# jketterl/digiham

Measured on AMD Instinct MI355X. Metric: concurrent 48 kS/s DMR channels sustained end-to-end (rrc_filter->gfsk_demodulator->dmr_decoder), higher is better.
Workload: dtype f32; 1 GPU; 16384 DMR channels/GPU x 3.96 s (190080 samples) of 48 kS/s FM-discriminator audio, full chain rrc(wide)->gfsk(10)->dmr_decoder incl. BPTC(196,96) (BASELINE con; channels_per_gpu=16384, total_channels=16384

## Files before the change

### digiham_amd/csrc/dsp_core.hpp

```cpp
#pragma once

#include "dh_portable.hpp"
#include "wave_ops.hpp"

#define DH_VARIANCE_SYMBOLS 100
#define DH_VOLUME_RB_SIZE 100
#define DH_FTILE 1024
#define DH_FIR_L 16
#define DH_PF_N 5
#define DH_PF_SINK 512
#define DH_MAX_NZ 160
#define DH_MAX_SPS 40
DH_HD uint32_t dh_history(uint32_t sps) { return DH_VARIANCE_SYMBOLS * (sps > 10u ? sps : 10u) + 152u; }
DH_HD uint32_t dh_tail_max(uint32_t sps) { return 256u + dh_history(sps); }
#define DH_STATE_HDR 32

enum { DH_ST_K = 0, DH_ST_OFF = 1, DH_ST_TAIL = 2, DH_ST_NSYM = 3, DH_ST_ORDERED = 4, DH_ST_BLOCKS = 5,
       DH_ST_P0 = 6,
       DH_ST_CUR_START = 7, DH_ST_CUR_OFF = 8, DH_ST_PREV_START = 9, DH_ST_PREV_OFF = 10,
       DH_ST_BLOCK_FLAGS = 11,
       DH_ST_E_CUR = 12, DH_ST_E_PREV = 13, DH_ST_E_COUNT = 14, DH_ST_E_BLOCK = 15,
       DH_ST_UNCERTAIN = 16, DH_ST_EXACT_RUNS = 17, DH_ST_EXACT_BLOCKS = 18,
       DH_ST_PART = 19,
       DH_ST_DIAG = 20 };
// ... 434 lines not shown
        }
    }
}
#else
template <int NZ, bool ONE>
inline void dh_fir_f16(const float* hw, const uint32_t (*G)[DH_WAVE][4], int lane, float k1, float k2, float* out16) {
    constexpr int DH_F16_KSTEPS = DH_F16_KSTEPS_OF(NZ), DH_F16_H2_OFFSET = DH_F16_H2_OFFSET_OF(NZ);
    const uint16_t* h1 = reinterpret_cast<const uint16_t*>(hw);
    const uint16_t* h2 = reinterpret_cast<const uint16_t*>(hw + DH_F16_H2_OFFSET);
    const int n = lane & 15, g = lane >> 4;
    for (int T = 0; T < 4; T++) for (int r = 0; r < 4; r++) {
        const uint32_t o = DH_F16_OUT(T, r, g, n), b16 = o - (uint32_t) n;
        float mn = 0.0f, sc = 0.0f;
        for (int i = 0; i < 3; i++) {
            const int pass = ONE ? (i == 0 ? 1 : i == 1 ? 0 : 2) : i;
            for (int s = 0; s < DH_F16_KSTEPS; s++) for (int qq = 0; qq < 4; qq++) for (int j = 0; j < 8; j++) {
                const int kk = 8 * qq + j;
                const uint32_t w = G[(pass == 1 ? DH_F16_KSTEPS : 0) + s][16 * qq + n][j >> 1];
                const float tap = dh_f16_value((uint16_t) (w >> (16 * (j & 1))));
                const uint16_t hv = (pass == 2 ? h2 : h1)[b16 + 32u * (uint32_t) s + (uint32_t) kk];
                if (pass == 0 && !ONE) mn = __builtin_fmaf(dh_f16_value(hv), tap, mn); else sc = __builtin_fmaf(dh_f16_value(hv), tap, sc);
            }
        }
        out16[4 * T + r] = ONE ? sc * k1 : __builtin_fmaf(sc, k2, mn * k1);
    }
}
#endif

DH_HD float dh_virtual_sample(const float* tail, uint32_t tc, const float* in, uint32_t idx) {
    return idx < tc ? tail[idx] : in[idx - tc];
}

struct DhAgcPair { float mn0, mx0, mn1, mx1; };

#if DH_ON_GPU
__device__ __forceinline__ void dh_agc_scan(DhDspShared& S, uint32_t k0, uint32_t k1, DH_LANE_STRUCT_REF(DhAgcPair, agc)) {
    const int lane = dh_fresh_lane_id_();
    const uint32_t e0 = 2u * (uint32_t) lane, e1 = e0 + 1u;
    const float c0 = e0 < k0 ? S.vol_old[e0] : S.vol_new[e0];
    const float c1 = e1 < k0 ? S.vol_old[e1] : S.vol_new[e1];
    const bool v0 = e0 < k1, v1 = e1 < k1;
    const float pmn0 = v0 ? c0 : DH_FLT_MAX, pmn1 = v1 ? c1 : DH_FLT_MAX;
    const float pmx0 = v0 ? c0 : DH_FLT_MIN, pmx1 = v1 ? c1 : DH_FLT_MIN;
    float pmn = dh_vmin(pmn0, pmn1), pmx = dh_vmax(pmx0, pmx1);
    const uint32_t r0 = 126u - e0, r1 = r0 + 1u;
    const float o0 = S.vol_old[r0], o1 = S.vol_old[r1];
    const float omn0 = r0 < DH_VOLUME_RB_SIZE ? o0 : DH_FLT_MAX, omn1 = r1 < DH_VOLUME_RB_SIZE ? o1 : DH_FLT_MAX;
    const float omx0 = r0 < DH_VOLUME_RB_SIZE ? o0 : DH_FLT_MIN, omx1 = r1 < DH_VOLUME_RB_SIZE ? o1 : DH_FLT_MIN;
    float smn = dh_vmin(omn0, omn1), smx = dh_vmax(omx0, omx1);
    dh_wave_prefix_minmax2(pmn, pmx, smn, smx);
    float epmn = DH_FLT_MAX, epmx = DH_FLT_MIN, esmn = DH_FLT_MAX, esmx = DH_FLT_MIN;
    dh_wave_prev4(epmn, epmx, esmn, esmx, pmn, pmx, smn, smx);
    const int from = (63 - lane) << 2;
    const float s1n = __int_as_float(__builtin_amdgcn_ds_bpermute(from, __float_as_int(esmn)));
    const float s1x = __int_as_float(__builtin_amdgcn_ds_bpermute(from, __float_as_int(esmx)));
    const float s0n = __int_as_float(__builtin_amdgcn_ds_bpermute(from, __float_as_int(dh_vmin(omn1, esmn))));
    const float s0x = __int_as_float(__builtin_amdgcn_ds_bpermute(from, __float_as_int(dh_vmax(omx1, esmx))));
    DhAgcPair r;
    r.mn0 = dh_vmin(dh_vmin(epmn, pmn0), s0n); r.mx0 = dh_vmax(dh_vmax(epmx, pmx0), s0x);
    r.mn1 = dh_vmin(pmn, s1n); r.mx1 = dh_vmax(pmx, s1x);
    S.mn[e0] = r.mn0; S.mx[e0] = r.mx0; S.mn[e1] = r.mn1; S.mx[e1] = r.mx1;
    agc = r;
}
#else
inline void dh_agc_scan(DhDspShared& S, uint32_t k0, uint32_t k1, DH_LANE_STRUCT_REF(DhAgcPair, agc)) {
    float pmn = DH_FLT_MAX, pmx = DH_FLT_MIN;
    for (uint32_t j = 0; j < k0; j++) { pmn = dh_fmin_(pmn, S.vol_old[j]); pmx = dh_fmax_(pmx, S.vol_old[j]); }
    for (uint32_t k = k0; k < k1; k++) {
        pmn = dh_fmin_(pmn, S.vol_new[k]); pmx = dh_fmax_(pmx, S.vol_new[k]);
        float smn = DH_FLT_MAX, smx = DH_FLT_MIN;
        for (uint32_t j = k + 1; j < DH_VOLUME_RB_SIZE; j++) { smn = dh_fmin_(smn, S.vol_old[j]); smx = dh_fmax_(smx, S.vol_old[j]); }
        S.mn[k] = dh_fmin_(pmn, smn); S.mx[k] = dh_fmax_(pmx, smx);
    }
    for (uint32_t l = 0; l < DH_WAVE; l++) {
        const uint32_t e0 = 2u * l, e1 = e0 + 1u, a = e0 >= k0 && e0 < k1 ? e0 : k0, b = e1 >= k0 && e1 < k1 ? e1 : k0;
        agc[l] = DhAgcPair{ S.mn[a], S.mx[a], S.mn[b], S.mx[b] };
    }
}
#endif

template <int NZ, bool FAST, int SPS> struct DhIsBounded {
    static constexpr bool value = !FAST && ((NZ == 80 && SPS == 10) || (NZ == 160 && SPS != 10));
};
#ifndef DH_STOP_AFTER
#define DH_STOP_AFTER 99
#endif
#define DH_BOUND_T_FACTOR 3.5f
#define DH_BOUND_XMAX_LO 1e-25f
#define DH_BOUND_XMAX_HI 1e15f

inline float dh_fir_error_coefficient(const float* taps_half, uint32_t nz, double gain) {
    double l1 = 0.0;
    for (uint32_t i = 0; i <= nz; i++) { const double c = taps_half[i <= nz / 2 ? i : nz - i]; l1 += c < 0 ? -c : c; }
    const double kappa = nz == 80 ? 240.0 : 1.44 * (2.0 * (nz + 1) + 5.0);
    const double coef = kappa * 5.9604644775390625e-08 * l1 / (gain < 0 ? -gain : gain) * 1.0001;
    float f = (float) coef;
    if ((double) f < coef) { union { float f; uint32_t u; } b; b.f = f; b.u++; f = b.f; }
    return f;
}

template <int NZ>
DH_HD float dh_exact_filtered(const float* tail, uint32_t tc, const float* in, uint32_t nv, const float* tapsf, double gain, double rgain, int32_t f) {
    if (f < 0 || (uint32_t) f + (uint32_t) NZ >= nv) return 0.0f;
    float acc = 0.0f;
// ... 182 lines not shown
            DH_FOR_LANES_FRESH(lane) {
                const uint32_t e = r * DH_WAVE + (uint32_t) lane;
                if (e < nj * nrows) {
                    uint32_t jj, i;
                    if (full) { jj = e / sps; i = e - jj * sps; }
                    else {
                        const uint32_t c = e / nj;
                        jj = e - c * nj;
                        uint64_t m = rows & all;
                        for (uint32_t b = 0; b < c; b++) m &= m - 1;
                        i = (uint32_t) dh_ffs64(m);
                    }
                    const uint32_t j = j0 + jj;
                    const int32_t f = C.cur_start + (int32_t) (j * sps) + (j ? C.cur_off : 0) + (int32_t) i;
                    S.var_rb[i * DH_VARIANCE_SYMBOLS + j] = dh_exact_filtered_lds<NZ>(stage, base, C.nv, C.tapsf, C.gain, C.rgain, f);
                }
            }
        }
    }
    DH_BARRIER();
}

template <int NZ>
DH_COLD void dh_exact_fir_pass(const DhDspParams& P, DhDspShared& S, uint32_t need, DH_LANE_ARRAY(float, (&fo), DH_FIR_L)) {
    float tv[NZ / 2 + 1];
    for (int i = 0; i <= NZ / 2; i++) tv[i] = S.tapsf[i];
    DH_FOR_LANES_FRESH(lane) {
        if ((uint32_t) (lane * DH_FIR_L) < need) {
            dh_fir_lane<NZ, false, false, true>(tv, P.gain, P.rgain, P.inv_gain, S.xf, lane, DH_LA(fo, lane));
        }
    }
}

template <int SPS>
DH_HD void dh_symbol_windows(DhDspShared& S, const float* fbuf, uint32_t k0, uint32_t m, int32_t step_off, uint32_t sps, uint32_t ev_lo, uint32_t ev_hi, float sps_rcp) {
#define DH_FB(n) fbuf[n]
    if (SPS == 10 && DH_STOP_AFTER >= 3) DH_FOR_LANES_FRESH(lane) {
        const uint32_t l = (uint32_t) lane;
        const uint32_t qa = l + 1u, qb = l < 35u ? l + 65u : 0u;
        const bool va = qa < m, vb = l < 35u ? qb < m : l == 35u;
        const float* srca = fbuf + (int32_t) (qa * 10u) + step_off;
        const float* srcb = l < 35u ? srca + 640 : fbuf;
        float v[10], w[10];
        dh_lds_run10_pair(srca, srcb, v, w);
        float vola = v[0], volb = w[0];
#pragma unroll
        for (int i = 1; i < 10; i++) { vola += v[i]; volb += w[i]; }
        const float mida = ((v[3] + v[4]) + v[5]) + v[6], midb = ((w[3] + w[4]) + w[5]) + w[6];
        const float volume_a = dh_div_const(vola, 10.0f, sps_rcp), volume_b = dh_div_const(volb, 10.0f, sps_rcp);
        if (va) {
            const uint32_t ka = k0 + qa;
            dh_lds_store_row10<0>(S.var_rb + ka, v[0], v[1], v[2], v[3], v[4], v[5], v[6], v[7], v[8], v[9]);
            S.sum[qa] = mida; S.vol_new[ka] = volume_a;
        }
        if (vb) {
            const uint32_t kb = k0 + qb;
            dh_lds_store_row10<0>(S.var_rb + kb, w[0], w[1], w[2], w[3], w[4], w[5], w[6], w[7], w[8], w[9]);
            S.sum[qb] = midb; S.vol_new[kb] = volume_b;
        }
        dh_lds_stores_done();
    }
    if (SPS == 20 && DH_STOP_AFTER >= 3) DH_FOR_LANES_FRESH(lane) {
        const uint32_t l = (uint32_t) lane;
        const uint32_t q = l < 63u ? l + 1u : 0u;
        const bool valid = q < m;
        const float* src = valid && q > 0u ? fbuf + (int32_t) (q * 20u) + step_off : fbuf;
        float v[20];
        dh_lds_run<20>(src, v);
        float vol = v[0];
#pragma unroll
        for (int i = 1; i < 20; i++) vol += v[i];
        const float mid = ((((v[7] + v[8]) + v[9]) + v[10]) + v[11]) + v[12];
        const float volume = dh_div_const(vol, 20.0f, sps_rcp);
        if (valid) {
            const uint32_t k = k0 + q;
            dh_lds_store_row10<0>(S.var_rb + k, v[0], v[1], v[2], v[3], v[4], v[5], v[6], v[7], v[8], v[9]);
            dh_lds_store_row10<1000>(S.var_rb + k, v[10], v[11], v[12], v[13], v[14], v[15], v[16], v[17], v[18], v[19]);
            S.sum[q] = mid; S.vol_new[k] = volume;
        }
        dh_lds_stores_done();
    }
    if (SPS == 40 && DH_STOP_AFTER >= 3) DH_FOR_LANES_FRESH(lane) {
        const uint32_t l = (uint32_t) lane;
        const uint32_t q = l < 63u ? l + 1u : 0u;
        const bool valid = q < m;
        const float* src = valid && q > 0u ? fbuf + (int32_t) (q * 40u) + step_off : fbuf;
        float v[40];
        dh_lds_run<40>(src, v);
        float vol = v[0], mid = v[13];
#pragma unroll
        for (int i = 1; i < 40; i++) vol += v[i];
#pragma unroll
        for (int i = 14; i < 27; i++) mid += v[i];
// ... 301 lines not shown
                        DH_BALLOT_ACC(v_above, l > hmin, lane);
                        DH_BALLOT_ACC(v_ok, DH_LA(iv_ok, lane)[0] != 0u, lane);
                        DH_BALLOT_ACC(v_pos, l > 0.0f, lane);
                        DH_BALLOT_ACC(v_small, h < 4999999.0f, lane);
                        DH_BALLOT_ACC(v_big, l > 5000001.0f, lane);
                    }
                    const uint64_t phases = sps >= 64u ? ~0ull : ((1ull << sps) - 1ull);
                    const uint64_t cand = ~v_above & phases;
                    const bool one = cand != 0 && (cand & (cand - 1)) == 0;
                    const bool sure = one && (v_ok & phases) == phases && (((v_pos & cand) && (v_small & cand)) || (v_big & cand));
                    if (!sure) continue;
                    DH_FOR_LANES_FRESH(lane) { if (DH_IS_LANE0(lane)) S.stats[1]++; }
                    const uint32_t vmin_pos = (uint32_t) dh_ffs64(cand);
                    if (v_big & cand) {
                    } else if (vmin_pos > 0 && vmin_pos < sps / 2) new_off = +1;
                    else if (vmin_pos >= sps / 2 && vmin_pos < sps - 1) new_off = -1;
                    break;
                }
                double vmin = S.variance[0]; uint32_t vmin_pos = 0;
                for (uint32_t i = 1; i < sps; i++) if (S.variance[i] < vmin) { vmin = S.variance[i]; vmin_pos = i; }
                DH_FOR_LANES_FRESH(lane) { if (DH_IS_LANE0(lane)) S.stats[1]++; }
                if (vmin <= 0 || vmin > 5000000) {
                } else if (vmin_pos > 0 && vmin_pos < sps / 2) new_off = +1;
                else if (vmin_pos >= sps / 2 && vmin_pos < sps - 1) new_off = -1;
                break;
            }
        }
    }
    return new_off;
}

struct DhSliceSetup { bool four_levels, e_pos, width_pow2, pair_store; float T_eff, inv_width; };
template <int SPS, int LV, bool BOUNDED>
DH_HD void dh_slice_symbols(const DhDspParams& P, DhDspShared& S, DH_LANE_STRUCT_IN(DhAgcPair, agc), uint8_t* out, uint32_t k0, uint32_t m, uint32_t ev_lo, uint32_t ev_hi,
                            const DhSliceSetup& U, uint64_t& vote_a, uint64_t& vote_b) {
    const bool four_levels = U.four_levels, e_pos = U.e_pos, width_pow2 = U.width_pow2, pair_store = U.pair_store;
    const float T_eff = U.T_eff, inv_width = U.inv_width;
    DH_FOR_LANES_FRESH(lane) {
        const uint32_t qa = 2u * (uint32_t) lane;
        const bool va = qa < m, vb = qa + 1u < m;
        const uint32_t qq = va ? qa : 0u, k = k0 + qq;
        const DhAgcPair& own = DH_LS(agc, lane);
        dh_f2 mn, mx;
        if (k0 == 0u) { mn = dh_f2_make(own.mn0, own.mn1); mx = dh_f2_make(own.mx0, own.mx1); }
        else { mn = dh_f2_make(S.mn[k], S.mn[k + 1u]); mx = dh_f2_make(S.mx[k], S.mx[k + 1u]); }
        const dh_f2 sumq = dh_f2_make(S.sum[qq], S.sum[qq + 1u]);
        const dh_f2 center = dh_f2_scale(dh_f2_add(mx, mn), 0.5f);
        const dh_f2 average = width_pow2 ? dh_f2_scale(sumq, inv_width) : SPS == 20 ? dh_div_const2(sumq, 6.0f, inv_width)
                                                                                    : dh_f2_make(sumq.x / (float) (ev_hi - ev_lo), sumq.y / (float) (ev_hi - ev_lo));
        const dh_f2 c625 = dh_f2_make(0.625f, 0.625f);
        const dh_f2 umid = dh_f2_fma(dh_f2_sub(mx, center), c625, center);
        const dh_f2 lmid = dh_f2_fma(dh_f2_sub(mn, center), c625, center);
        const bool above_a = average.x > center.x, above_b = average.y > center.y;
        const uint8_t sym4a = above_a ? (average.x > umid.x ? 1 : 0) : (average.x < lmid.x ? 3 : 2);
        const uint8_t sym4b = above_b ? (average.y > umid.y ? 1 : 0) : (average.y < lmid.y ? 3 : 2);
        const uint8_t sym2a = LV == 4 ? (uint8_t) 0 : above_a ? (uint8_t) !P.invert : (uint8_t) (P.invert != 0);
        const uint8_t sym2b = LV == 4 ? (uint8_t) 0 : above_b ? (uint8_t) !P.invert : (uint8_t) (P.invert != 0);
        const uint8_t sa = four_levels ? sym4a : sym2a, sb = four_levels ? sym4b : sym2b;
        bool doubt_a = false, doubt_b = false;
        if (BOUNDED) {
            const dh_f2 du = dh_f2_sub(average, umid), dl = dh_f2_sub(average, lmid), dc = dh_f2_sub(average, center);
            const float da = dh_min3_abs(four_levels ? du.x : DH_FLT_MAX, four_levels ? dl.x : DH_FLT_MAX, dc.x);
            const float db = dh_min3_abs(four_levels ? du.y : DH_FLT_MAX, four_levels ? dl.y : DH_FLT_MAX, dc.y);
            doubt_a = va && e_pos && !(da > T_eff);
            doubt_b = vb && e_pos && !(db > T_eff);
        }
#ifdef DH_IGNORE_DOUBT
        doubt_a = false; doubt_b = false;
#endif
        if (DH_LIKELY(pair_store)) {
            if (vb) *reinterpret_cast<uint16_t*>(out + qa) = (uint16_t) ((uint32_t) sa | ((uint32_t) sb << 8));
            if (DH_UNLIKELY((m & 1u) != 0u)) { if (qa + 1u == m) out[qa] = sa; }
        } else {
            if (va) out[qa] = sa;
            if (vb) out[qa + 1u] = sb;
        }
        DH_BALLOT_ACC(vote_a, doubt_a, lane);
        DH_BALLOT_ACC(vote_b, doubt_b, lane);
    }
// ... 439 lines not shown
        DH_TAPFRAG_SETTLE(tapfrag_regs, NFRAG, MF16);
        DH_PHASE_MARK(1);
        const float* fbuf = S.xf;

        const uint32_t p_next = last_start + sps + ((k0 == 0 && m == 1) ? (uint32_t) step_off : 0u);
        const uint32_t pf_have = dh_min<uint32_t>(DH_FTILE + NZ, nv - p_next);
        DH_LANE_ARRAY(dh_f4, pfr, PF_REG ? DH_PF_N : 1);
        const bool pf_plain = p_next - tc < pf_lim;
        const bool pf_reg = PF_REG && pf_plain && P.exact_mode != 2;
        if constexpr (KEEPF) {
            const uint32_t f_lo = tc > (uint32_t) NZ ? tc - (uint32_t) NZ : 0u;
            const uint32_t s0 = p < f_lo ? f_lo - p : 0u;
            const uint32_t s1 = dh_min<uint32_t>(p_next - p, nf > p ? nf - p : 0u);
            float* orow = P.filt_out + (size_t) ch * P.filt_stride + ((ptrdiff_t) p + (ptrdiff_t) NZ - (ptrdiff_t) tc);
            DH_FOR_LANES_FRESH(lane) {
                for (uint32_t e = s0 + (uint32_t) lane; e < s1; e += DH_WAVE) orow[e] = fbuf[e];
            }
        }

        DH_COMPILER_FENCE();
        float e_blk = 0.0f;
        if (BOUNDED) { e_blk = dh_uniform_f(__builtin_fmaxf(e_blk_run, e_run)); e_blk_run = e_blk; }
        const float e_eff = BOUNDED ? dh_uniform_f(__builtin_fmaxf(e_run, __builtin_fmaxf(e_cur, e_prev))) : 0.0f;
        const float T = DH_BOUND_T_FACTOR * e_eff;
        uint64_t vote_a = 0, vote_b = 0;
        const bool four_levels = LV ? LV == 4 : P.levels == 4;
        const bool force_doubt = BOUNDED && P.exact_mode == 1;
        const bool e_pos = e_eff > 0.0f || force_doubt;
        const float T_eff = force_doubt ? __builtin_inff() : T;
        const float inv_width = 1.0f / (float) (ev_hi - ev_lo);
        const bool width_pow2 = ((ev_hi - ev_lo) & (ev_hi - ev_lo - 1u)) == 0u;
        const bool pair_store = ((uint32_t) (uintptr_t) syms + nsym) % 2u == 0u;

        dh_symbol_windows<SPS>(S, fbuf, k0, m, step_off, sps, ev_lo, ev_hi, sps_rcp);
        DH_BARRIER();
        DH_PHASE_MARK(2);

        dh_issue_next_window<NZ, PF_REG>(S, in, tc, p_next, pf_plain, pf_reg, pfr);

        DH_LANE_STRUCT(DhAgcPair, agc) = {};
        if (DH_STOP_AFTER >= 4) dh_agc_scan(S, k0, k0 + m, agc);
        DH_BARRIER();
        DH_PHASE_MARK(3);

        if (DH_STOP_AFTER >= 5) {
            const DhSliceSetup U = { four_levels, e_pos, width_pow2, pair_store, T_eff, inv_width };
            dh_slice_symbols<SPS, LV, BOUNDED>(P, S, agc, syms + nsym, k0, m, ev_lo, ev_hi, U, vote_a, vote_b);
        }
        if (BOUNDED && DH_UNLIKELY((vote_a | vote_b) != 0)) {
            dh_settle_doubts<NZ>(P, S, BS, V, syms + nsym, k0, e_eff, sps, ev_lo, ev_hi, vote_a, vote_b);
        }

        DH_PHASE_MARK(4);
        int32_t new_off = 0;
        const bool block_done = (k0 + m == DH_VARIANCE_SYMBOLS);
        if (block_done && DH_STOP_AFTER >= 6) {
            new_off = dh_timing_decision<NZ, SPS, BOUNDED>(P, S, BS, V, sps, k0, e_blk);
        }

        DH_PHASE_MARK(5);
        DH_FOR_LANES_FRESH(lane) {
            const uint32_t ka = k0 + (uint32_t) lane, kb = ka + DH_WAVE, ke = k0 + m;
            const uint32_t ia = ka < ke ? ka : k0, ib = kb < ke ? kb : k0;
            const float va_ = S.vol_new[ia], vb_ = S.vol_new[ib];
            S.vol_old[ia] = va_;
            S.vol_old[ib] = vb_;
        }
        staged_p = 0xFFFFFFFFu;
        if (DH_LIKELY(pf_reg)) {
            if constexpr (PF_REG && MF16) { if (DH_LIKELY((dh_stage_f16<NZ, ONE_CHAIN>(P, S, pfr, pf_have, st_e_run, st_k1, st_k2)))) staged_p = p_next; }
            else if constexpr (PF_PLAIN) {
                static_assert(!PF_PLAIN || (DH_FTILE == 4u * DH_WAVE * (DH_PF_N - 1)), "four full groups cover the window");
                DH_FOR_LANES_FRESH(lane) {
                    const uint32_t l4 = 4u * (uint32_t) lane;
                    float* ldst = &S.xf[l4];
#pragma unroll
                    for (int r = 0; r < DH_PF_N - 1; r++) {
                        dh_f4 w = DH_LA(pfr, lane)[PF_REG ? r : 0];
                        if (DH_UNLIKELY(pf_have < DH_FTILE)) w = dh_zero_beyond(w, l4 + 4u * DH_WAVE * (uint32_t) r, pf_have);
                        dh_store4(ldst + 4 * DH_WAVE * r, w);
// ... 185 lines not shown
```

### digiham_amd/csrc/wave_ops.hpp

```cpp
#pragma once

#include "dh_portable.hpp"

#define DH_FLT_MAX 3.402823466e+38f
#define DH_DBL_MAX 1.7976931348623157e+308
#define DH_FLT_MIN 1.175494351e-38f

#if DH_ON_GPU
typedef float dh_f2 __attribute__((ext_vector_type(2)));
typedef float dh_v4f __attribute__((ext_vector_type(4)));
typedef float dh_f32x4 __attribute__((ext_vector_type(4)));
typedef _Float16 dh_h8 __attribute__((ext_vector_type(8)));
typedef _Float16 dh_h4 __attribute__((ext_vector_type(4)));
typedef uint32_t dh_u4 __attribute__((ext_vector_type(4)));
#else
struct dh_f2 { float x, y; };
typedef uint16_t dh_h4[4];
#endif
struct __attribute__((aligned(4))) dh_f4 { float x, y, z, w; };
struct alignas(16) dh_f4a { float x, y, z, w; };
DH_HD dh_f4 dh_load4_unaligned(const float* p) { dh_f4 v; __builtin_memcpy(&v, p, sizeof(v)); return v; }
DH_HD void dh_store4(float* q, const dh_f4& v) { q[0] = v.x; q[1] = v.y; q[2] = v.z; q[3] = v.w; }
DH_HD void dh_store4_unaligned(float* q, const dh_f4& v) { __builtin_memcpy(q, &v, sizeof(v)); }

// ... 144 lines not shown
    dh_v4f xs; xs.x = v.x; xs.y = v.y; xs.z = v.z; xs.w = v.w;
    xs = xs * scale;
    const dh_h4 a = __builtin_convertvector(xs, dh_h4);
    const dh_v4f af = __builtin_convertvector(a, dh_v4f);
    const dh_f2 x01 = xs.xy, x23 = xs.zw, a01 = af.xy, a23 = af.zw;
    dh_f2 r01, r23;
    asm("v_pk_add_f32 %0, %1, %2 neg_lo:[0,1] neg_hi:[0,1]" : "=v"(r01) : "v"(x01), "v"(a01));
    asm("v_pk_add_f32 %0, %1, %2 neg_lo:[0,1] neg_hi:[0,1]" : "=v"(r23) : "v"(x23), "v"(a23));
    dh_v4f r; r.xy = r01; r.zw = r23;
    h1 = a; h2 = __builtin_convertvector(r, dh_h4);
#else
    const float x[4] = { v.x, v.y, v.z, v.w };
    for (int i = 0; i < 4; i++) {
        const float xs = x[i] * scale;
        h1[i] = dh_f16_bits(xs);
        h2[i] = dh_f16_bits(xs - dh_f16_value(h1[i]));
    }
#endif
}
DH_HD void dh_h4_store(dh_h4* dst, const dh_h4& v) { __builtin_memcpy(dst, &v, sizeof(dh_h4)); }

#if DH_ON_GPU
template <int O0, int O1> __device__ __forceinline__ dh_f2 dh_lds_read2(uint32_t addr) {
    static_assert(O0 < 256 && O1 < 256, "ds_read2_b32 offsets are 8-bit dword counts");
    dh_f2 v;
    asm volatile("ds_read2_b32 %0, %1 offset0:%2 offset1:%3" : "=v"(v) : "v"(addr), "n"(O0), "n"(O1) : "memory");
    return v;
}
template <int OFF_BYTES> __device__ __forceinline__ dh_f2 dh_lds_read_b64(uint32_t addr) {
    dh_f2 v;
    asm volatile("ds_read_b64 %0, %1 offset:%2" : "=v"(v) : "v"(addr), "n"(OFF_BYTES) : "memory");
    return v;
}
template <int OFF_BYTES> __device__ __forceinline__ dh_v4f dh_lds_read_b128(uint32_t addr) {
    dh_v4f v;
    asm volatile("ds_read_b128 %0, %1 offset:%2" : "=v"(v) : "v"(addr), "n"(OFF_BYTES) : "memory");
    return v;
}
#endif
template <int N> DH_HD void dh_lds_run(const float* src, float (&v)[N]) {
#if DH_ON_GPU
    static_assert(N == 20 || N == 40, "five or ten 16-byte reads");
    const uint32_t a = (uint32_t) (uintptr_t) (const __attribute__((address_space(3))) float*) src;
    dh_v4f x0 = dh_lds_read_b128<0>(a), x1 = dh_lds_read_b128<16>(a), x2 = dh_lds_read_b128<32>(a), x3 = dh_lds_read_b128<48>(a), x4 = dh_lds_read_b128<64>(a);
    if constexpr (N == 20) {
        asm volatile("s_waitcnt lgkmcnt(0)" : "+v"(x0), "+v"(x1), "+v"(x2), "+v"(x3), "+v"(x4) :: "memory");
        v[0] = x0.x; v[1] = x0.y; v[2] = x0.z; v[3] = x0.w; v[4] = x1.x; v[5] = x1.y; v[6] = x1.z; v[7] = x1.w; v[8] = x2.x; v[9] = x2.y;
        v[10] = x2.z; v[11] = x2.w; v[12] = x3.x; v[13] = x3.y; v[14] = x3.z; v[15] = x3.w; v[16] = x4.x; v[17] = x4.y; v[18] = x4.z; v[19] = x4.w;
    } else {
        dh_v4f x5 = dh_lds_read_b128<80>(a), x6 = dh_lds_read_b128<96>(a), x7 = dh_lds_read_b128<112>(a), x8 = dh_lds_read_b128<128>(a), x9 = dh_lds_read_b128<144>(a);
        asm volatile("s_waitcnt lgkmcnt(0)" : "+v"(x0), "+v"(x1), "+v"(x2), "+v"(x3), "+v"(x4), "+v"(x5), "+v"(x6), "+v"(x7), "+v"(x8), "+v"(x9) :: "memory");
        const dh_v4f x[10] = { x0, x1, x2, x3, x4, x5, x6, x7, x8, x9 };
#pragma unroll
        for (int i = 0; i < 10; i++) { v[4 * i] = x[i].x; v[4 * i + 1] = x[i].y; v[4 * i + 2] = x[i].z; v[4 * i + 3] = x[i].w; }
    }
#else
    for (int i = 0; i < N; i++) v[i] = src[i];
#endif
}
DH_HD void dh_lds_run10_pair(const float* srca, const float* srcb, float (&v)[10], float (&w)[10]) {
#if DH_ON_GPU
    const uint32_t aa = (uint32_t) (uintptr_t) (const __attribute__((address_space(3))) float*) srca;
    const uint32_t ab = (uint32_t) (uintptr_t) (const __attribute__((address_space(3))) float*) srcb;
    dh_f2 x0 = dh_lds_read_b64<0>(aa), x1 = dh_lds_read_b64<8>(aa), x2 = dh_lds_read_b64<16>(aa), x3 = dh_lds_read_b64<24>(aa), x4 = dh_lds_read_b64<32>(aa);
    dh_f2 y0 = dh_lds_read_b64<0>(ab), y1 = dh_lds_read_b64<8>(ab), y2 = dh_lds_read_b64<16>(ab), y3 = dh_lds_read_b64<24>(ab), y4 = dh_lds_read_b64<32>(ab);
    asm volatile("s_waitcnt lgkmcnt(0)" : "+v"(x0), "+v"(x1), "+v"(x2), "+v"(x3), "+v"(x4), "+v"(y0), "+v"(y1), "+v"(y2), "+v"(y3), "+v"(y4) :: "memory");
    v[0] = x0.x; v[1] = x0.y; v[2] = x1.x; v[3] = x1.y; v[4] = x2.x; v[5] = x2.y; v[6] = x3.x; v[7] = x3.y; v[8] = x4.x; v[9] = x4.y;
    w[0] = y0.x; w[1] = y0.y; w[2] = y1.x; w[3] = y1.y; w[4] = y2.x; w[5] = y2.y; w[6] = y3.x; w[7] = y3.y; w[8] = y4.x; w[9] = y4.y;
#else
    for (int i = 0; i < 10; i++) { v[i] = srca[i]; w[i] = srcb[i]; }
#endif
}

#if DH_ON_GPU
template <int OFF_WORDS> __device__ __forceinline__ void dh_lds_store4_at(float* base, const dh_f4& v) {
    static_assert(4 * OFF_WORDS + 12 < 65536, "ds_write_b32 offsets are 16-bit byte counts");
    const uint32_t addr = (uint32_t) (uintptr_t) (__attribute__((address_space(3))) float*) base;
    asm volatile("ds_write_b32 %0, %1 offset:%5\n\tds_write_b32 %0, %2 offset:%6\n\tds_write_b32 %0, %3 offset:%7\n\tds_write_b32 %0, %4 offset:%8"
                 :: "v"(addr), "v"(v.x), "v"(v.y), "v"(v.z), "v"(v.w), "n"(4 * OFF_WORDS), "n"(4 * OFF_WORDS + 4), "n"(4 * OFF_WORDS + 8), "n"(4 * OFF_WORDS + 12) : "memory");
}
__device__ __forceinline__ void dh_lds_stores_done() { asm volatile("s_waitcnt lgkmcnt(0)" ::: "memory"); }
template <int K> __device__ __forceinline__ void dh_lds_store_row10(float* base, float a0, float a1, float a2, float a3, float a4, float a5, float a6, float a7, float a8, float a9) {
    const uint32_t addr = (uint32_t) (uintptr_t) (__attribute__((address_space(3))) float*) base;
    asm volatile("ds_write_b32 %0, %1 offset:%11\n\tds_write_b32 %0, %2 offset:%12\n\tds_write_b32 %0, %3 offset:%13\n\tds_write_b32 %0, %4 offset:%14\n\t"
                 "ds_write_b32 %0, %5 offset:%15\n\tds_write_b32 %0, %6 offset:%16\n\tds_write_b32 %0, %7 offset:%17\n\tds_write_b32 %0, %8 offset:%18\n\t"
                 "ds_write_b32 %0, %9 offset:%19\n\tds_write_b32 %0, %10 offset:%20"
                 :: "v"(addr), "v"(a0), "v"(a1), "v"(a2), "v"(a3), "v"(a4), "v"(a5), "v"(a6), "v"(a7), "v"(a8), "v"(a9),
                    "n"(4 * K), "n"(4 * (K + 100)), "n"(4 * (K + 200)), "n"(4 * (K + 300)), "n"(4 * (K + 400)), "n"(4 * (K + 500)), "n"(4 * (K + 600)),
                    "n"(4 * (K + 700)), "n"(4 * (K + 800)), "n"(4 * (K + 900)) : "memory");
}
#else
template <int OFF_WORDS> inline void dh_lds_store4_at(float* base, const dh_f4& v) { dh_store4(base + OFF_WORDS, v); }
inline void dh_lds_stores_done() {}
template <int K> inline void dh_lds_store_row10(float* base, float a0, float a1, float a2, float a3, float a4, float a5, float a6, float a7, float a8, float a9) {
    const float a[10] = { a0, a1, a2, a3, a4, a5, a6, a7, a8, a9 };
    for (int i = 0; i < 10; i++) base[i * 100 + K] = a[i];
}
#endif

DH_HD void dh_l2_touch_lines(const float* base, uint32_t n, float* sink) {
#if DH_ON_GPU
    const uint32_t pf_lane = (uint32_t) dh_fresh_lane_id_();
    const float* line = base + 32u * pf_lane;
    const uint32_t sink_addr = (uint32_t) (uintptr_t) (__attribute__((address_space(3))) float*) sink;
    uint32_t keep_m0;
    if (32u * pf_lane < n)
        asm volatile("s_mov_b32 %0, m0\n\ts_mov_b32 m0, %1\n\tglobal_load_lds_dword %2, off\n\ts_mov_b32 m0, %0"
                     : "=&s"(keep_m0) : "s"(sink_addr), "v"(line) : "memory");
#endif
}
DH_HD void dh_global_loads_done() { DH_GPU_ELSE(asm volatile("s_waitcnt vmcnt(0)" ::: "memory"), (void) 0); }

#if DH_ON_GPU
#define DH_TAPFRAG_REGS(name, N, table) dh_u4 name[N]
#define DH_TAPFRAG_LOAD(name, N, table, on) do { if constexpr (on) { const dh_u4* tf_ = reinterpret_cast<const dh_u4*>(table) + dh_fresh_lane_id_(); \
        _Pragma("unroll") for (int f_ = 0; f_ < (N); f_++) name[f_] = tf_[DH_WAVE * f_]; } } while (0)
#define DH_TAPFRAG_SETTLE(name, N, on) do { if constexpr (on) { _Pragma("unroll") for (int f_ = 0; f_ < (N); f_++) \
        asm volatile("" :: "v"(name[f_])); } } while (0)
#else
#define DH_TAPFRAG_REGS(name, N, table) const uint32_t (* const name)[DH_WAVE][4] = reinterpret_cast<const uint32_t (*)[DH_WAVE][4]>(table)
#define DH_TAPFRAG_LOAD(name, N, table, on) ((void) 0)
#define DH_TAPFRAG_SETTLE(name, N, on) ((void) 0)
#endif

#if DH_ON_GPU
__device__ __forceinline__ void dh_wave_prefix_minmax2(float& mn, float& mx, float& mn2, float& mx2) {
// ... 103 lines not shown
```

Baseline: 13.98 million channels.

## Keep SPS10 symbol windows in lane registers, drop barriers before AGC scan and slicing

For the 10-samples-per-symbol path, each lane now handles two adjacent symbols from one contiguous 20-sample LDS read and keeps their volume, mid-sum and matching old-volume values in registers. These feed the AGC scan and the slicer directly, so the two block barriers between window, AGC and slice stages are removed. Stores are merged into paired ds_write2 instructions. This adds a cold shift of symbol 0 when step_off is nonzero and fallback LDS reads when k0 is not zero, and correctness now depends on lane ownership matching across the stages.

```diff
diff --git a/digiham_amd/csrc/dsp_core.hpp b/digiham_amd/csrc/dsp_core.hpp
--- a/digiham_amd/csrc/dsp_core.hpp
+++ b/digiham_amd/csrc/dsp_core.hpp
@@ -490,19 +490,30 @@
 }
 
 struct DhAgcPair { float mn0, mx0, mn1, mx1; };
+struct DhWinPair { float vol0, vol1, sum0, sum1, old0, old1; };
 
 #if DH_ON_GPU
-__device__ __forceinline__ void dh_agc_scan(DhDspShared& S, uint32_t k0, uint32_t k1, DH_LANE_STRUCT_REF(DhAgcPair, agc)) {
+template <bool PAIRS>
+__device__ __forceinline__ void dh_agc_scan(DhDspShared& S, uint32_t k0, uint32_t k1, DH_LANE_STRUCT_REF(DhAgcPair, agc), DH_LANE_STRUCT_IN(DhWinPair, win), bool from_win) {
     const int lane = dh_fresh_lane_id_();
     const uint32_t e0 = 2u * (uint32_t) lane, e1 = e0 + 1u;
-    const float c0 = e0 < k0 ? S.vol_old[e0] : S.vol_new[e0];
-    const float c1 = e1 < k0 ? S.vol_old[e1] : S.vol_new[e1];
+    float c0, c1;
+    if (!PAIRS) { c0 = e0 < k0 ? S.vol_old[e0] : S.vol_new[e0]; c1 = e1 < k0 ? S.vol_old[e1] : S.vol_new[e1]; }
+    else if (DH_LIKELY(from_win)) { c0 = win.vol0; c1 = win.vol1; }
+    else {
+        c0 = dh_lds_read_b32<0>(dh_lds_addr((e0 < k0 ? S.vol_old : S.vol_new) + e0));
+        c1 = dh_lds_read_b32<0>(dh_lds_addr((e1 < k0 ? S.vol_old : S.vol_new) + e1));
+        dh_lds_reads_done(c0, c1);
+    }
     const bool v0 = e0 < k1, v1 = e1 < k1;
     const float pmn0 = v0 ? c0 : DH_FLT_MAX, pmn1 = v1 ? c1 : DH_FLT_MAX;
     const float pmx0 = v0 ? c0 : DH_FLT_MIN, pmx1 = v1 ? c1 : DH_FLT_MIN;
     float pmn = dh_vmin(pmn0, pmn1), pmx = dh_vmax(pmx0, pmx1);
     const uint32_t r0 = 126u - e0, r1 = r0 + 1u;
-    const float o0 = S.vol_old[r0], o1 = S.vol_old[r1];
+    float o0, o1;
+    if (!PAIRS) { o0 = S.vol_old[r0]; o1 = S.vol_old[r1]; }
+    else if (DH_LIKELY(from_win)) { o0 = win.old0; o1 = win.old1; }
+    else { o0 = dh_lds_read_b32<0>(dh_lds_addr(S.vol_old + r0)); o1 = dh_lds_read_b32<0>(dh_lds_addr(S.vol_old + r1)); dh_lds_reads_done(o0, o1); }
     const float omn0 = r0 < DH_VOLUME_RB_SIZE ? o0 : DH_FLT_MAX, omn1 = r1 < DH_VOLUME_RB_SIZE ? o1 : DH_FLT_MAX;
     const float omx0 = r0 < DH_VOLUME_RB_SIZE ? o0 : DH_FLT_MIN, omx1 = r1 < DH_VOLUME_RB_SIZE ? o1 : DH_FLT_MIN;
     float smn = dh_vmin(omn0, omn1), smx = dh_vmax(omx0, omx1);
@@ -521,13 +532,18 @@
     agc = r;
 }
 #else
-inline void dh_agc_scan(DhDspShared& S, uint32_t k0, uint32_t k1, DH_LANE_STRUCT_REF(DhAgcPair, agc)) {
+template <bool PAIRS>
+inline void dh_agc_scan(DhDspShared& S, uint32_t k0, uint32_t k1, DH_LANE_STRUCT_REF(DhAgcPair, agc), DH_LANE_STRUCT_IN(DhWinPair, win), bool from_win) {
     float pmn = DH_FLT_MAX, pmx = DH_FLT_MIN;
     for (uint32_t j = 0; j < k0; j++) { pmn = dh_fmin_(pmn, S.vol_old[j]); pmx = dh_fmax_(pmx, S.vol_old[j]); }
     for (uint32_t k = k0; k < k1; k++) {
-        pmn = dh_fmin_(pmn, S.vol_new[k]); pmx = dh_fmax_(pmx, S.vol_new[k]);
+        const float vk = !from_win ? S.vol_new[k] : (k & 1u) ? win[k >> 1].vol1 : win[k >> 1].vol0;
+        pmn = dh_fmin_(pmn, vk); pmx = dh_fmax_(pmx, vk);
         float smn = DH_FLT_MAX, smx = DH_FLT_MIN;
-        for (uint32_t j = k + 1; j < DH_VOLUME_RB_SIZE; j++) { smn = dh_fmin_(smn, S.vol_old[j]); smx = dh_fmax_(smx, S.vol_old[j]); }
+        for (uint32_t j = k + 1; j < DH_VOLUME_RB_SIZE; j++) {
+            const float oj = !from_win ? S.vol_old[j] : (j & 1u) ? win[(127u - j) >> 1].old1 : win[(126u - j) >> 1].old0;
+            smn = dh_fmin_(smn, oj); smx = dh_fmax_(smx, oj);
+        }
         S.mn[k] = dh_fmin_(pmn, smn); S.mx[k] = dh_fmax_(pmx, smx);
     }
     for (uint32_t l = 0; l < DH_WAVE; l++) {
@@ -776,33 +792,43 @@
     }
 }
 
+DH_COLD void dh_shift_symbol0(float* fbuf, int32_t step_off) {
+    DH_LANE_VALUE(float, t);
+    DH_FOR_LANES_FRESH(lane) { DH_LV(t, lane) = fbuf[lane < 10 ? lane : 0]; }
+    DH_FOR_LANES_FRESH(lane) { if (lane < 10) fbuf[lane + step_off] = DH_LV(t, lane); }
+}
+
 template <int SPS>
-DH_HD void dh_symbol_windows(DhDspShared& S, const float* fbuf, uint32_t k0, uint32_t m, int32_t step_off, uint32_t sps, uint32_t ev_lo, uint32_t ev_hi, float sps_rcp) {
+DH_HD void dh_symbol_windows(DhDspShared& S, const float* fbuf, uint32_t k0, uint32_t m, int32_t step_off, uint32_t sps, uint32_t ev_lo, uint32_t ev_hi, float sps_rcp,
+                             DH_LANE_STRUCT_REF(DhWinPair, win)) {
 #define DH_FB(n) fbuf[n]
     if (SPS == 10 && DH_STOP_AFTER >= 3) DH_FOR_LANES_FRESH(lane) {
         const uint32_t l = (uint32_t) lane;
-        const uint32_t qa = l + 1u, qb = l < 35u ? l + 65u : 0u;
-        const bool va = qa < m, vb = l < 35u ? qb < m : l == 35u;
-        const float* srca = fbuf + (int32_t) (qa * 10u) + step_off;
-        const float* srcb = l < 35u ? srca + 640 : fbuf;
-        float v[10], w[10];
-        dh_lds_run10_pair(srca, srcb, v, w);
+        const uint32_t qa = 2u * l, qb = qa + 1u;
+        const bool vb = qb < m;
+        const float* src = l < 50u ? fbuf + (int32_t) (l * 20u) + step_off : fbuf;
+        float x[20], v[10], w[10], old0, old1;
+        dh_lds_run20_with_pair(src, x, S.vol_old + (126u - qa), old0, old1);
+#pragma unroll
+        for (int i = 0; i < 10; i++) { v[i] = x[i]; w[i] = x[10 + i]; }
         float vola = v[0], volb = w[0];
 #pragma unroll
         for (int i = 1; i < 10; i++) { vola += v[i]; volb += w[i]; }
-        const float mida = ((v[3] + v[4]) + v[5]) + v[6], midb = ((w[3] + w[4]) + w[5]) + w[6];
+        float mida = v[3] + v[4]; DH_TO_VGPR(mida); mida += v[5]; DH_TO_VGPR(mida); mida += v[6]; DH_TO_VGPR(mida);
+        const float midb = ((w[3] + w[4]) + w[5]) + w[6];
         const float volume_a = dh_div_const(vola, 10.0f, sps_rcp), volume_b = dh_div_const(volb, 10.0f, sps_rcp);
-        if (va) {
-            const uint32_t ka = k0 + qa;
-            dh_lds_store_row10<0>(S.var_rb + ka, v[0], v[1], v[2], v[3], v[4], v[5], v[6], v[7], v[8], v[9]);
-            S.sum[qa] = mida; S.vol_new[ka] = volume_a;
-        }
+        const uint32_t ka = k0 + qa;
         if (vb) {
-            const uint32_t kb = k0 + qb;
-            dh_lds_store_row10<0>(S.var_rb + kb, w[0], w[1], w[2], w[3], w[4], w[5], w[6], w[7], w[8], w[9]);
-            S.sum[qb] = midb; S.vol_new[kb] = volume_b;
-        }
-        dh_lds_stores_done();
+            dh_lds_store_rows10_pair(S.var_rb + ka, v, w);
+            dh_lds_store_pair(S.sum + qa, mida, midb); dh_lds_store_pair(S.vol_new + ka, volume_a, volume_b);
+        }
+        if (DH_UNLIKELY((m & 1u) != 0u)) {
+            if (qb == m) {
+                dh_lds_store_row10<0>(S.var_rb + ka, v[0], v[1], v[2], v[3], v[4], v[5], v[6], v[7], v[8], v[9]);
+                S.sum[qa] = mida; S.vol_new[ka] = volume_a;
+            }
+        }
+        DH_LS(win, lane) = DhWinPair{ volume_a, volume_b, mida, midb, old0, old1 };
     }
     if (SPS == 20 && DH_STOP_AFTER >= 3) DH_FOR_LANES_FRESH(lane) {
         const uint32_t l = (uint32_t) lane;
@@ -1170,7 +1196,7 @@
 
 struct DhSliceSetup { bool four_levels, e_pos, width_pow2, pair_store; float T_eff, inv_width; };
 template <int SPS, int LV, bool BOUNDED>
-DH_HD void dh_slice_symbols(const DhDspParams& P, DhDspShared& S, DH_LANE_STRUCT_IN(DhAgcPair, agc), uint8_t* out, uint32_t k0, uint32_t m, uint32_t ev_lo, uint32_t ev_hi,
+DH_HD void dh_slice_symbols(const DhDspParams& P, DhDspShared& S, DH_LANE_STRUCT_IN(DhAgcPair, agc), DH_LANE_STRUCT_IN(DhWinPair, win), uint8_t* out, uint32_t k0, uint32_t m, uint32_t ev_lo, uint32_t ev_hi,
                             const DhSliceSetup& U, uint64_t& vote_a, uint64_t& vote_b) {
     const bool four_levels = U.four_levels, e_pos = U.e_pos, width_pow2 = U.width_pow2, pair_store = U.pair_store;
     const float T_eff = U.T_eff, inv_width = U.inv_width;
@@ -1179,10 +1205,16 @@
         const bool va = qa < m, vb = qa + 1u < m;
         const uint32_t qq = va ? qa : 0u, k = k0 + qq;
         const DhAgcPair& own = DH_LS(agc, lane);
-        dh_f2 mn, mx;
-        if (k0 == 0u) { mn = dh_f2_make(own.mn0, own.mn1); mx = dh_f2_make(own.mx0, own.mx1); }
-        else { mn = dh_f2_make(S.mn[k], S.mn[k + 1u]); mx = dh_f2_make(S.mx[k], S.mx[k + 1u]); }
-        const dh_f2 sumq = dh_f2_make(S.sum[qq], S.sum[qq + 1u]);
+        const DhWinPair& own_win = DH_LS(win, lane);
+        dh_f2 mn, mx, sumq;
+        if (SPS == 10) {
+            if (DH_LIKELY(k0 == 0u)) { mn = dh_f2_make(own.mn0, own.mn1); mx = dh_f2_make(own.mx0, own.mx1); sumq = dh_f2_make(own_win.sum0, own_win.sum1); }
+            else dh_lds_pairs3_now(S.mn + k, S.mx + k, S.sum + qq, mn, mx, sumq);
+        } else {
+            if (k0 == 0u) { mn = dh_f2_make(own.mn0, own.mn1); mx = dh_f2_make(own.mx0, own.mx1); }
+            else { mn = dh_f2_make(S.mn[k], S.mn[k + 1u]); mx = dh_f2_make(S.mx[k], S.mx[k + 1u]); }
+            sumq = dh_f2_make(S.sum[qq], S.sum[qq + 1u]);
+        }
         const dh_f2 center = dh_f2_scale(dh_f2_add(mx, mn), 0.5f);
         const dh_f2 average = width_pow2 ? dh_f2_scale(sumq, inv_width) : SPS == 20 ? dh_div_const2(sumq, 6.0f, inv_width)
                                                                                     : dh_f2_make(sumq.x / (float) (ev_hi - ev_lo), sumq.y / (float) (ev_hi - ev_lo));
@@ -1688,20 +1720,22 @@
         const bool width_pow2 = ((ev_hi - ev_lo) & (ev_hi - ev_lo - 1u)) == 0u;
         const bool pair_store = ((uint32_t) (uintptr_t) syms + nsym) % 2u == 0u;
 
-        dh_symbol_windows<SPS>(S, fbuf, k0, m, step_off, sps, ev_lo, ev_hi, sps_rcp);
-        DH_BARRIER();
+        DH_LANE_STRUCT(DhWinPair, win) = {};
+        if (SPS == 10 && DH_STOP_AFTER >= 3 && DH_UNLIKELY(step_off != 0)) dh_shift_symbol0(S.xf, step_off);
+        dh_symbol_windows<SPS>(S, fbuf, k0, m, step_off, sps, ev_lo, ev_hi, sps_rcp, win);
+        if (SPS != 10) DH_BARRIER();
         DH_PHASE_MARK(2);
 
         dh_issue_next_window<NZ, PF_REG>(S, in, tc, p_next, pf_plain, pf_reg, pfr);
 
         DH_LANE_STRUCT(DhAgcPair, agc) = {};
-        if (DH_STOP_AFTER >= 4) dh_agc_scan(S, k0, k0 + m, agc);
-        DH_BARRIER();
+        if (DH_STOP_AFTER >= 4) dh_agc_scan<SPS == 10>(S, k0, k0 + m, agc, win, SPS == 10 && k0 == 0u);
+        if (SPS != 10) DH_BARRIER();
         DH_PHASE_MARK(3);
 
         if (DH_STOP_AFTER >= 5) {
             const DhSliceSetup U = { four_levels, e_pos, width_pow2, pair_store, T_eff, inv_width };
-            dh_slice_symbols<SPS, LV, BOUNDED>(P, S, agc, syms + nsym, k0, m, ev_lo, ev_hi, U, vote_a, vote_b);
+            dh_slice_symbols<SPS, LV, BOUNDED>(P, S, agc, win, syms + nsym, k0, m, ev_lo, ev_hi, U, vote_a, vote_b);
         }
         if (BOUNDED && DH_UNLIKELY((vote_a | vote_b) != 0)) {
             dh_settle_doubts<NZ>(P, S, BS, V, syms + nsym, k0, e_eff, sps, ev_lo, ev_hi, vote_a, vote_b);
diff --git a/digiham_amd/csrc/wave_ops.hpp b/digiham_amd/csrc/wave_ops.hpp
--- a/digiham_amd/csrc/wave_ops.hpp
+++ b/digiham_amd/csrc/wave_ops.hpp
@@ -200,6 +200,13 @@
     asm volatile("ds_read_b64 %0, %1 offset:%2" : "=v"(v) : "v"(addr), "n"(OFF_BYTES) : "memory");
     return v;
 }
+template <int OFF_BYTES> __device__ __forceinline__ float dh_lds_read_b32(uint32_t addr) {
+    float v;
+    asm volatile("ds_read_b32 %0, %1 offset:%2" : "=v"(v) : "v"(addr), "n"(OFF_BYTES) : "memory");
+    return v;
+}
+__device__ __forceinline__ void dh_lds_reads_done(float& a, float& b) { asm volatile("s_waitcnt lgkmcnt(0)" : "+v"(a), "+v"(b) :: "memory"); }
+__device__ __forceinline__ uint32_t dh_lds_addr(const float* p) { return (uint32_t) (uintptr_t) (const __attribute__((address_space(3))) float*) p; }
 template <int OFF_BYTES> __device__ __forceinline__ dh_v4f dh_lds_read_b128(uint32_t addr) {
     dh_v4f v;
     asm volatile("ds_read_b128 %0, %1 offset:%2" : "=v"(v) : "v"(addr), "n"(OFF_BYTES) : "memory");
@@ -226,17 +233,25 @@
     for (int i = 0; i < N; i++) v[i] = src[i];
 #endif
 }
-DH_HD void dh_lds_run10_pair(const float* srca, const float* srcb, float (&v)[10], float (&w)[10]) {
-#if DH_ON_GPU
-    const uint32_t aa = (uint32_t) (uintptr_t) (const __attribute__((address_space(3))) float*) srca;
-    const uint32_t ab = (uint32_t) (uintptr_t) (const __attribute__((address_space(3))) float*) srcb;
-    dh_f2 x0 = dh_lds_read_b64<0>(aa), x1 = dh_lds_read_b64<8>(aa), x2 = dh_lds_read_b64<16>(aa), x3 = dh_lds_read_b64<24>(aa), x4 = dh_lds_read_b64<32>(aa);
-    dh_f2 y0 = dh_lds_read_b64<0>(ab), y1 = dh_lds_read_b64<8>(ab), y2 = dh_lds_read_b64<16>(ab), y3 = dh_lds_read_b64<24>(ab), y4 = dh_lds_read_b64<32>(ab);
-    asm volatile("s_waitcnt lgkmcnt(0)" : "+v"(x0), "+v"(x1), "+v"(x2), "+v"(x3), "+v"(x4), "+v"(y0), "+v"(y1), "+v"(y2), "+v"(y3), "+v"(y4) :: "memory");
-    v[0] = x0.x; v[1] = x0.y; v[2] = x1.x; v[3] = x1.y; v[4] = x2.x; v[5] = x2.y; v[6] = x3.x; v[7] = x3.y; v[8] = x4.x; v[9] = x4.y;
-    w[0] = y0.x; w[1] = y0.y; w[2] = y1.x; w[3] = y1.y; w[4] = y2.x; w[5] = y2.y; w[6] = y3.x; w[7] = y3.y; w[8] = y4.x; w[9] = y4.y;
-#else
-    for (int i = 0; i < 10; i++) { v[i] = srca[i]; w[i] = srcb[i]; }
+DH_HD void dh_lds_run20_with_pair(const float* src, float (&v)[20], const float* pair, float& p0, float& p1) {
+#if DH_ON_GPU
+    dh_f2 q = dh_lds_read_b64<0>((uint32_t) (uintptr_t) (const __attribute__((address_space(3))) float*) pair);
+    dh_lds_run<20>(src, v);
+    asm volatile("s_waitcnt lgkmcnt(0)" : "+v"(q) :: "memory");
+    p0 = q.x; p1 = q.y;
+#else
+    dh_lds_run<20>(src, v);
+    p0 = pair[0]; p1 = pair[1];
+#endif
+}
+DH_HD void dh_lds_pairs3_now(const float* pa, const float* pb, const float* pc, dh_f2& a, dh_f2& b, dh_f2& c) {
+#if DH_ON_GPU
+    a = dh_lds_read2<0, 1>((uint32_t) (uintptr_t) (const __attribute__((address_space(3))) float*) pa);
+    b = dh_lds_read2<0, 1>((uint32_t) (uintptr_t) (const __attribute__((address_space(3))) float*) pb);
+    c = dh_lds_read2<0, 1>((uint32_t) (uintptr_t) (const __attribute__((address_space(3))) float*) pc);
+    asm volatile("s_waitcnt lgkmcnt(0)" : "+v"(a), "+v"(b), "+v"(c) :: "memory");
+#else
+    a = dh_f2_make(pa[0], pa[1]); b = dh_f2_make(pb[0], pb[1]); c = dh_f2_make(pc[0], pc[1]);
 #endif
 }
 
@@ -257,9 +272,28 @@
                     "n"(4 * K), "n"(4 * (K + 100)), "n"(4 * (K + 200)), "n"(4 * (K + 300)), "n"(4 * (K + 400)), "n"(4 * (K + 500)), "n"(4 * (K + 600)),
                     "n"(4 * (K + 700)), "n"(4 * (K + 800)), "n"(4 * (K + 900)) : "memory");
 }
+__device__ __forceinline__ void dh_lds_store_pair(float* base, float a, float b) {
+    const uint32_t addr = (uint32_t) (uintptr_t) (__attribute__((address_space(3))) float*) base;
+    asm volatile("ds_write2_b32 %0, %1, %2 offset1:1" :: "v"(addr), "v"(a), "v"(b) : "memory");
+}
+__device__ __forceinline__ void dh_lds_store_rows3_pair_(uint32_t addr, float a0, float b0, float a1, float b1, float a2, float b2) {
+    asm volatile("ds_write2_b32 %0, %1, %2 offset1:1\n\tds_write2_b32 %0, %3, %4 offset0:100 offset1:101\n\tds_write2_b32 %0, %5, %6 offset0:200 offset1:201"
+                 :: "v"(addr), "v"(a0), "v"(b0), "v"(a1), "v"(b1), "v"(a2), "v"(b2) : "memory");
+}
+__device__ __forceinline__ void dh_lds_store_rows10_pair(float* base, const float (&a)[10], const float (&b)[10]) {
+    const uint32_t addr = (uint32_t) (uintptr_t) (__attribute__((address_space(3))) float*) base;
+    dh_lds_store_rows3_pair_(addr, a[0], b[0], a[1], b[1], a[2], b[2]);
+    dh_lds_store_rows3_pair_(addr + 1200u, a[3], b[3], a[4], b[4], a[5], b[5]);
+    dh_lds_store_rows3_pair_(addr + 2400u, a[6], b[6], a[7], b[7], a[8], b[8]);
+    asm volatile("ds_write2_b32 %0, %1, %2 offset1:1" :: "v"(addr + 3600u), "v"(a[9]), "v"(b[9]) : "memory");
+}
 #else
 template <int OFF_WORDS> inline void dh_lds_store4_at(float* base, const dh_f4& v) { dh_store4(base + OFF_WORDS, v); }
 inline void dh_lds_stores_done() {}
+inline void dh_lds_store_pair(float* base, float a, float b) { base[0] = a; base[1] = b; }
+inline void dh_lds_store_rows10_pair(float* base, const float (&a)[10], const float (&b)[10]) {
+    for (int i = 0; i < 10; i++) { base[i * 100] = a[i]; base[i * 100 + 1] = b[i]; }
+}
 template <int K> inline void dh_lds_store_row10(float* base, float a0, float a1, float a2, float a3, float a4, float a5, float a6, float a7, float a8, float a9) {
     const float a[10] = { a0, a1, a2, a3, a4, a5, a6, a7, a8, a9 };
     for (int i = 0; i < 10; i++) base[i * 100 + K] = a[i];
```

After: 14.34 million channels, median of 6. +2.5%, better.
